# gregorgebhardt/gym-kilobots

Measured on AMD Instinct MI355X. Metric: kilobot-steps/sec, higher is better.
Workload: dtype f32

## Files before the change

gym_kilobots_amd/csrc/kb_regsolve_bins.inc:

```
{
    constexpr int KRB = KB_KREG_BINS;
    const bool solving = (int)__builtin_amdgcn_readfirstlane(wave) < nsolve;
    unsigned ra[KRB], rb[KRB], rm[KRB];
    float racc[KRB], rnx[KRB], rny[KRB];
    const unsigned WOFF = 8u * (unsigned)(NB - 5);
    char *const velB = reinterpret_cast<char *>(vel), *const posB = reinterpret_cast<char *>(pos);
#define RB_WALL(j) (ra[j] >= WOFF)
#define RB_WALLIDX(j) ((int)((ra[j] - WOFF) >> 3))
#define RB_VEL(off) (*reinterpret_cast<float2 *>(velB + (off)))
#define RB_POS(off) (*reinterpret_cast<float2 *>(posB + (off)))
#define RB_C(j) ((int)(rm[j] & 0xFFFu))
#define RB_DEPTH(j) ((int)((rm[j] >> 12) & 0x1FFu))
#define RB_FLIP(j) (((rm[j] >> 21) & 1u) != 0u)
#define RB_ISL(j) ((int)(rm[j] >> 22))
#pragma unroll
    for (int j = 0; j < KRB; ++j) { ra[j] = 0u; rb[j] = 0u; rm[j] = 0u; racc[j] = 0.0f; rnx[j] = 1.0f; rny[j] = 0.0f; }
    unsigned long long slotLevels[KRB];
    int dlo[KRB], dhi[KRB];
#pragma unroll
    for (int j = 0; j < KRB; ++j) { slotLevels[j] = 0ull; dlo[j] = 1; dhi[j] = 0; }
    int maxD = 0;
    unsigned mycnt = 0;
    const float nm_bb = p.nm_bb, nm_wb = p.nm_wb;
#ifdef KB_SOLVER_PRIO
// ... 54 lines not shown
            if (mycnt > 64u) { rlo = wave_or(rlo); rhi = wave_or(rhi); restmask = ((unsigned long long)rhi << 32) | rlo; }
        }
        wave_sync();
#ifdef KB_PROFILE
        if (tid == 0) { atomicAdd(&KB_PROF(8), (unsigned)__popcll(keymask)); atomicAdd(&KB_PROF(11), 1u); }
#endif
        KB_STAMP_PRE(19);
        unsigned *bodyDepth = islCnt;
        {
            char *const bdB = reinterpret_cast<char *>(bodyDepth);
#define RB_BD(off) (*reinterpret_cast<unsigned *>(bdB + (off)))
            unsigned rc[KRB], ia4[KRB], ib4[KRB];
#pragma unroll
            for (int j = 0; j < KRB; ++j) {
                const unsigned key = lk[j] & 63u, r = (lk[j] >> 8) & 0xFFu;
                const bool on = (lk[j] >> 31) != 0u && key != 63u;
                rc[j] = on ? ((key % RK) == RK - 1 ? (key | (r << 6)) : key) : 0xFFFFFFFFu;
                ib4[j] = 4u * (unsigned)RB_B(j);
                ia4[j] = RB_A(j) < WALL_CODE ? 4u * (unsigned)RB_A(j) : ib4[j];
            }
            const unsigned mrow = bkMaxRank[wave * NUM_CLS + min((int)lane, NUM_CLS - 1)];
            for (unsigned long long m_ = keymask; m_; m_ &= m_ - 1) {
                const unsigned key_ = (unsigned)__builtin_ctzll(m_);
                const bool rest_ = ((restmask >> key_) & 1ull) != 0ull;
                auto depth_round = [&](unsigned code_) __attribute__((always_inline)) {
#pragma unroll
                    for (int j = 0; j < KRB; ++j) {
                        if (j == 0 || rest_) {
                            if (rc[j] == code_) {
                                const unsigned d = max(RB_BD(ia4[j]), RB_BD(ib4[j])) + 1u;
                                rdepth[j] = (int)d;
                                RB_BD(ib4[j]) = d;
                                RB_BD(ia4[j]) = d;
                            }
                        }
                    }
                    wave_sync();
                };
                if ((key_ % RK) < RK - 1) depth_round(key_);
                else {
                    const unsigned maxr_ = (unsigned)__builtin_amdgcn_readlane((int)mrow, (int)(key_ / RK));
                    for (unsigned r_ = RK - 1; r_ <= maxr_; ++r_) depth_round(key_ | (r_ << 6));
                }
            }
#undef RB_BD
        }
#pragma unroll
        for (int j = 0; j < KRB; ++j) maxD = max(maxD, rdepth[j]);
        maxD = (int)wave_umax((unsigned)maxD);
        KB_STAMP_PRE(20);
        if (mycnt > 64u) {
            unsigned at[KRB];
#pragma unroll
            for (int j = 0; j < KRB; ++j) at[j] = 0u;
            unsigned base_ = 0;
            for (int d_ = SLEEP ? 0 : 1; d_ <= maxD; ++d_) {
#pragma unroll
                for (int j = 0; j < KRB; ++j) {
                    const bool is = (lk[j] >> 31) && rdepth[j] == d_;
                    const unsigned long long m_ = __ballot(is);
                    const unsigned mine = __builtin_amdgcn_mbcnt_hi((unsigned)(m_ >> 32), __builtin_amdgcn_mbcnt_lo((unsigned)m_, base_));
                    at[j] = is ? mine : at[j];
                    base_ += (unsigned)__popcll(m_);
                }
            }
#pragma unroll
            for (int j = 0; j < KRB; ++j)
                if (lk[j] >> 31) {
                    lOrder[mybase + at[j]] = (unsigned short)((lk[j] >> 16) & 0xFFFu);
                    lCbk[mybase + at[j]] = (unsigned short)rdepth[j];
                }
            wave_sync();
            unsigned short o_[KRB], l_[KRB];
#pragma unroll
            for (int j = 0; j < KRB; ++j) {
                const unsigned i_ = mybase + ((lk[j] >> 31) ? lane + 64u * j : 0u);
                o_[j] = lOrder[i_]; l_[j] = lCbk[i_];
            }
#pragma unroll
            for (int j = 0; j < KRB; ++j) {
                const bool v_ = (lk[j] >> 31) != 0u;
                lk[j] = v_ ? ((lk[j] & 0x8000FFFFu) | ((unsigned)o_[j] << 16)) : lk[j];
                rdepth[j] = v_ ? (int)l_[j] : rdepth[j];
            }
        }
        KB_STAMP_PRE(21);
#pragma unroll
        for (int j = 0; j < KRB; ++j) {
            const unsigned long long mine = (lk[j] >> 31) ? 1ull << min(rdepth[j], 63) : 0ull;
            const unsigned lo = wave_or((unsigned)mine), hi = wave_or((unsigned)(mine >> 32));
            slotLevels[j] = ((unsigned long long)hi << 32) | (unsigned long long)lo;
            const unsigned long long lv = slotLevels[j] >> 1;
            dlo[j] = lv ? (int)__builtin_ctzll(lv) + 1 : 1;
            dhi[j] = lv ? ((lv >> 62) ? maxD : 64 - (int)__builtin_clzll(lv)) : 0;
        }
        {
            unsigned c_[KRB], pr_[KRB], inf_[KRB], root_[KRB];
            float acc_[KRB];
            float2 pa_[KRB], pb_[KRB];
            bool v_[KRB];
#pragma unroll
            for (int j = 0; j < KRB; ++j) {
                v_[j] = (lk[j] >> 31) != 0u;
                c_[j] = v_[j] ? (lk[j] >> 16) & 0xFFFu : 0u;
                pr_[j] = lPair[c_[j]]; inf_[j] = lInfo[c_[j]]; acc_[j] = lAcc[c_[j]];
            }
#pragma unroll
            for (int j = 0; j < KRB; ++j) {
                pr_[j] = v_[j] ? pr_[j] : 0u;
                const int a = (int)(pr_[j] & 0xFFFFu), b = (int)(pr_[j] >> 16);
                pa_[j] = pos[a >= WALL_CODE ? b : a]; pb_[j] = pos[b]; root_[j] = parent[b];
            }
            bool pairOn[KRB];
            float dx[KRB], dy[KRB], dd[KRB], wnx[KRB], wny[KRB];
            bool ieee = false;
#pragma unroll
            for (int j = 0; j < KRB; ++j) {
                const int a = (int)(pr_[j] & 0xFFFFu), b = (int)(pr_[j] >> 16);
                const bool wallA = a >= WALL_CODE, flip = (inf_[j] & 0x80u) != 0u;
                ra[j] = wallA ? WOFF + 8u * (unsigned)(a - WALL_CODE) : 8u * (unsigned)a;
                rb[j] = 8u * (unsigned)b;
                racc[j] = v_[j] ? acc_[j] : 0.0f;
                rm[j] = v_[j] ? (c_[j] | ((unsigned)rdepth[j] << 12) | (flip ? 1u << 21 : 0u) | (root_[j] << 22)) : 0u;
                float dist;
                wall_geom(p, wallA ? a - WALL_CODE : 0, pb_[j].x, pb_[j].y, dist, wnx[j], wny[j]);
                if (flip) { wnx[j] = -wnx[j]; wny[j] = -wny[j]; }
                dx[j] = pb_[j].x - pa_[j].x; dy[j] = pb_[j].y - pa_[j].y;
                dd[j] = dx[j] * dx[j] + dy[j] * dy[j];
                pairOn[j] = v_[j] && !wallA && dd[j] > B2_EPSILON * B2_EPSILON;
                ieee = ieee || (pairOn[j] && !kb_exact_guard(dd[j]));
                if (wallA) { rnx[j] = wnx[j]; rny[j] = wny[j]; } else { rnx[j] = 1.0f; rny[j] = 0.0f; }
            }
            if (__builtin_expect(__builtin_amdgcn_ballot_w64(ieee) == 0ull, 1)) {
#pragma unroll
                for (int j = 0; j < KRB; ++j) {
                    const float len = kb_sqrt_refine(dd[j], __builtin_amdgcn_sqrtf(dd[j]), __builtin_amdgcn_rsqf(dd[j]));
                    const float inv = kb_rcp_refine(len, __builtin_amdgcn_rcpf(len));
                    if (pairOn[j]) { rnx[j] = dx[j] * inv; rny[j] = dy[j] * inv; }
                }
            } else {
#pragma unroll
                for (int j = 0; j < KRB; ++j) {
                    const float len = sqrtf(dd[j]);
                    const float inv = 1.0f / len;
                    if (pairOn[j]) { rnx[j] = dx[j] * inv; rny[j] = dy[j] * inv; }
                }
            }
        }
#undef RB_A
#undef RB_B
#ifdef KB_PROFILE
        if (lane == 0) atomicMax(&misc[M_PROF], (unsigned)maxD);
        if (tid == 0) atomicAdd(&KB_PROF(M_PROF_DEPTH), (unsigned)maxD);
        KB_STAMP(7);
#endif
    }
    KB_ABLATE_EXIT(9);
#define RB_ON(j) (RB_DEPTH(j) == d_)
    if (solving) {
#pragma unroll
        for (int j = 0; j < KRB; ++j) {
            for (int d_ = dlo[j]; d_ <= dhi[j]; ++d_) {
                if (RB_ON(j)) {
                    const float2 va = RB_VEL(ra[j]), vb = RB_VEL(rb[j]);
                    const float Px = racc[j] * rnx[j], Py = racc[j] * rny[j];
                    const float ima = RB_WALL(j) ? 0.0f : p.im_bot;
                    RB_VEL(ra[j]) = make_float2(va.x - ima * Px, va.y - ima * Py);
                    RB_VEL(rb[j]) = make_float2(vb.x + p.im_bot * Px, vb.y + p.im_bot * Py);
                }
                wave_sync();
            }
        }
        KB_STAMP_PRE(29);
    }
    KB_ABLATE_EXIT(10);
    if (solving) {
        for (int it = 0; it < p.vel_iters; ++it) {
#pragma unroll
            for (int j = 0; j < KRB; ++j) {
                for (int d_ = dlo[j]; d_ <= dhi[j]; ++d_) {
                    if (RB_ON(j)) {
                        const float2 va = RB_VEL(ra[j]), vb = RB_VEL(rb[j]);
                        const bool wallA = RB_WALL(j);
                        const float nx = rnx[j], ny = rny[j];
                        const float ima = wallA ? 0.0f : p.im_bot, imb = p.im_bot;
                        const float dvx = vb.x - va.x, dvy = vb.y - va.y;
                        const float vn = dvx * nx + dvy * ny;
                        float lambda = -((wallA ? nm_wb : nm_bb) * vn);
                        const float accOld = racc[j];
                        const float newimp = fmaxf(accOld + lambda, 0.0f);
                        lambda = newimp - accOld;
                        racc[j] = newimp;
                        const float Px = lambda * nx, Py = lambda * ny;
                        RB_VEL(ra[j]) = make_float2(va.x - ima * Px, va.y - ima * Py);
                        RB_VEL(rb[j]) = make_float2(vb.x + imb * Px, vb.y + imb * Py);
                    }
                    wave_sync();
                }
            }
        }
        KB_STAMP_PRE(30);
    }
    KB_STAMP(4);
    KB_RETID();
    KB_ABLATE_EXIT(11);
    if (solving) {
#pragma unroll
        for (int j = 0; j < KRB; ++j)
            if (lane + 64u * j < mycnt) lAcc[RB_C(j)] = racc[j];
    }
    {
        const unsigned char unsolved = (unsigned char)(p.pos_iters <= 0 ? 1 : 0);
        char *const sxB = reinterpret_cast<char *>(startX), *const syB = reinterpret_cast<char *>(startY);
        auto integrate_xy = [&](const unsigned off8, const float2 v0, const float2 p0) __attribute__((always_inline)) {
            float vxx = v0.x, vyy = v0.y;
            *reinterpret_cast<float *>(sxB + (off8 >> 1)) = p0.x; *reinterpret_cast<float *>(syB + (off8 >> 1)) = p0.y;
            const float tx = h * vxx, ty = h * vyy;
            if (tx * tx + ty * ty > B2_MAX_TRANSLATION_SQ) {
                const float ratio = B2_MAX_TRANSLATION / sqrtf(tx * tx + ty * ty);
                vxx *= ratio; vyy *= ratio;
            }
            RB_POS(off8) = make_float2(p0.x + h * vxx, p0.y + h * vyy);
            RB_VEL(off8) = make_float2(vxx, vyy);
        };
        bool intA[KRB], intB[KRB], own[BPT];
        {
            unsigned dA[KRB], dB[KRB], mk[BPT];
            const char *const bdB = reinterpret_cast<const char *>(islCnt);
#pragma unroll
            for (int j = 0; j < KRB; ++j) {
                dA[j] = *reinterpret_cast<const unsigned *>(bdB + ((RB_WALL(j) ? rb[j] : ra[j]) >> 1));
                dB[j] = *reinterpret_cast<const unsigned *>(bdB + (rb[j] >> 1));
            }
#pragma unroll
            for (int q = 0; q < BPT; ++q) mk[q] = intMark[(unsigned)ms[q] & 31u];
#pragma unroll
            for (int j = 0; j < KRB; ++j) {
                const unsigned d = (unsigned)RB_DEPTH(j);
                intA[j] = solving && d != 0u && !RB_WALL(j) && dA[j] == d;
                intB[j] = solving && d != 0u && dB[j] == d;
            }
#pragma unroll
            for (int q = 0; q < BPT; ++q) {
                own[q] = tid + q * nt < N && ((mk[q] >> ((unsigned)ms[q] >> 5)) & 1u) == 0u;
            }
        }
        wave_sync();
        static_assert(KRB == BPT, "a register slot and a kilobot of the owner thread share a trip");
#pragma unroll
        for (int j = 0; j < KRB; ++j) {
            const unsigned oo = 8u * (unsigned)ms[j];
            const float2 vO = RB_VEL(oo), pO = RB_POS(oo);
            const unsigned char aO = SLEEP ? active[ms[j]] : (unsigned char)1;
            if (j == 0 || mycnt > 64u) {
                const float2 vA = RB_VEL(ra[j]), vB = RB_VEL(rb[j]), pA = RB_POS(ra[j]), pB = RB_POS(rb[j]);
                if (intA[j]) {
                    integrate_xy(ra[j], vA, pA);
                    if (SLEEP) islWave[ra[j] >> 3] = (unsigned char)(2 | unsolved);
                }
                if (intB[j]) {
                    integrate_xy(rb[j], vB, pB);
                    if (SLEEP) islWave[rb[j] >> 3] = (unsigned char)(2 | unsolved);
                }
            }
            if (own[j]) {
                integrate_xy(oo, vO, pO);
                if (SLEEP) islWave[ms[j]] = (unsigned char)((aO ? 2 : 0) | unsolved);
            }
            float ww = bw[j];
            const float rot = h * ww;
            if (rot * rot > B2_MAX_ROTATION_SQ) {
                const float ratio = B2_MAX_ROTATION / fabsf(rot);
                ww *= ratio;
            }
            th[j] += h * ww;
            bw[j] = ww;
        }
    }
    wave_sync();
    KB_STAMP(5);
    KB_ABLATE_EXIT(12);
    if (solving) {
        for (int it = 0; it < p.pos_iters; ++it) {
            unsigned char *act = active + (it & 1) * NB, *nxt = active + ((it + 1) & 1) * NB;
            bool viol = false;
            bool ron[KRB];
#pragma unroll
            for (int j = 0; j < KRB; ++j) ron[j] = (lane + 64u * j < mycnt) && act[RB_ISL(j)] != 0;
#pragma unroll
            for (int j = 0; j < KRB; ++j) {
                for (int d_ = dlo[j]; d_ <= dhi[j]; ++d_) {
                    if (ron[j] && RB_ON(j)) {
                    const bool wallA = RB_WALL(j);
                    const int isl = RB_ISL(j);
                    float nx, ny, sep;
                    const float ima = wallA ? 0.0f : p.im_bot, imb = p.im_bot;
                    const float2 pb = RB_POS(rb[j]);
                    const float bx = pb.x, by = pb.y;
                    float axx = 0.0f, ayy = 0.0f;
                    if (wallA) {
                        float dist, wx, wy;
                        wall_geom(p, RB_WALLIDX(j), bx, by, dist, wx, wy);
                        nx = RB_FLIP(j) ? -wx : wx; ny = RB_FLIP(j) ? -wy : wy;
                        const float along = RB_FLIP(j) ? -dist : dist;
                        sep = along - B2_POLYGON_RADIUS - p.r_bot;
                    } else {
// ... 50 lines not shown
```

gym_kilobots_amd/csrc/kb_step_kernel.h:

```cpp
#pragma once
#include <utility>

#include "kb_common.h"
#include "kb_objects.h"

namespace kb {

template <int DRIVE_MODE, int LIGHT_TYPE, bool OBJ, int FN = 0, int TIER = 0, bool POLY = true, bool SENSE = true, bool SLEEP = false>
__global__ void __launch_bounds__(TIER == 1 ? 64 : 64 * KB_MAX_WAVES, (TIER == 1 || TIER == 3) ? 2 : ((TIER == 2 || (FN != 0 && !OBJ)) ? KB_COMPACT_WAVES_PER_SIMD : KB_MIN_WAVES_PER_SIMD)) kb_step_kernel(const Params p) {
    constexpr bool WIDE = TIER == 1 || TIER == 3;
    constexpr bool BINS = !OBJ;
    constexpr int KRX = BINS ? KB_KREG_BINS : KREG;
    constexpr bool PAR_DS = FN != 0 && BINS;
    static_assert(!SLEEP || FN == 0 || !OBJ, "the fixed-size instantiations with objects do not carry the sleep state");
    extern __shared__ __align__(16) unsigned char smem[];
    {
        static_assert(sizeof(Params) >= 6 * 64, "the six lines asked for are kernel arguments");
        const __attribute__((address_space(4))) unsigned *ka_ = (const __attribute__((address_space(4))) unsigned *)__builtin_amdgcn_kernarg_segment_ptr();
        const __attribute__((address_space(1))) unsigned char *m_ = (const __attribute__((address_space(1))) unsigned char *)p.env_mask;
        asm volatile("" : "+s"(m_) : "s"(ka_[0]), "s"(ka_[16]), "s"(ka_[32]), "s"(ka_[48]), "s"(ka_[64]), "s"(ka_[80]));
        if (m_ && !m_[blockIdx.x]) return;
    }
    int e = blockIdx.x;
    int tid = threadIdx.x;
// ... 934 lines not shown
                        for (int w2 = 0; w2 < 3; ++w2) {
                            float dist, nx, ny;
                            wall_geom(p, w2, ax, ay, dist, nx, ny);
                            if (w2 < wl && !(dist * dist > rw2)) r++;
                        }
                        cls = CLS_WALL | (int)(inf0 & 0x80u);
                        slot = nbots + r;
                        acc = ws_find(a, (unsigned)(WALL_CODE + wl));
                    } else {
                        const int a = pr & 0xFFFF;
                        const unsigned b = pr >> 16;
                        const int cell = cellOf[a];
                        const int cx = cell % p.gw, cy = cell / p.gw;
                        const float ax = pos[a].x, ay = pos[a].y;
                        if (k == 0) cls = CLS_SAME;
                        else if (k == 1) cls = CLS_E + (cx & 1);
                        else if (k == 2) cls = CLS_N + (cy & 1);
                        else if (k == 3) cls = CLS_NE + (cx & 1);
                        else cls = CLS_NW + (cx & 1);
                        const unsigned dc = dirCnt[a];
                        int sbase = 0;
                        for (int k2 = 0; k2 < k; ++k2) sbase += (int)((dc >> (6 * k2)) & 63u);
                        int rbase = 0;
                        for (unsigned a2 = head[hix(cell)]; a2 != (unsigned)EMPTY16; a2 = nextb[a2])
                            if ((int)a2 < a && (!hashed || (int)cellOf[a2] == cell)) rbase += (int)((dirCnt[a2] >> (6 * k)) & 63u);
                        int j = 0;
                        if (((dc >> (6 * k)) & 63u) > 1u) {
                            const int oc = (cy + dir_dy(k)) * p.gw + (cx + dir_dx(k));
                            for (unsigned b2 = head[hix(oc)]; b2 != (unsigned)EMPTY16; b2 = nextb[b2]) {
                                if (b2 >= b || (k == 0 && (int)b2 <= a) || (hashed && (int)cellOf[b2] != oc)) continue;
                                const float2 pb2 = pos[b2];
                                const float ex = pb2.x - ax, ey = pb2.y - ay;
                                if (!(ex * ex + ey * ey > rr2)) j++;
                            }
                        }
                        r = rbase + j;
                        slot = sbase + j;
                        acc = ws_find(a, b);
                        if (acc < 0.0f) acc = ws_find((int)b, (unsigned)a);
                        unsigned ra = a, rb = b;
                        for (;;) {
                            while (true) { unsigned t = lds_load_relaxed<PAR_DS>(&parent[ra]); if (t == ra) break; ra = t; }
                            while (true) { unsigned t = lds_load_relaxed<PAR_DS>(&parent[rb]); if (t == rb) break; rb = t; }
                            if (ra == rb) break;
                            if (ra < rb) { unsigned t = ra; ra = rb; rb = t; }
                            if (atomicCAS(&parent[ra], ra, rb) == ra) break;
                        }
                    }
                    if (acc < 0.0f) acc = 0.0f;
                    if (slot >= S) slot = 255;
                    if (r > 255) { r = 255; atomicOr(&misc[M_STATUS], 4u); }
                    sInfo[c] = (unsigned)cls | ((unsigned)r << 8) | ((unsigned)slot << 16) | fixbits;
                    sAcc[c] = acc;
                }
            };
            if (big) label_pass(gPair, gInfo, gAcc); else label_pass(lPair, lInfo, lAcc);
            KB_STAMP_PRE(18);
            __syncthreads();
            KB_STAMP(2);
            KB_RETID();

        }

        if (SLEEP) {
#pragma unroll
            for (int q = 0; q < BPT; ++q) {
                const int b = tid + q * nt;
                if (b >= N) continue;
                const int cnt = wsCnt[b], off = wsOff[b];
                for (int s_ = 0; s_ < cnt && off + s_ < p.cap; ++s_) {
                    const float a_ = oldInLds ? oldAcc[off + s_] : g.ws_acc[wo + off + s_];
                    if (a_ < 0.0f) continue;
                    unsigned key = oldInLds ? (unsigned)oldKey[off + s_] : g.ws_key[wo + off + s_];
                    if (!oldInLds) key = key >= KEY_OBJ ? OBJ_CODE + (key - KEY_OBJ) : (key >= KEY_WALL ? WALL_CODE + (key - KEY_WALL) : key);
                    if (key >= (unsigned)WALL_CODE) continue;
                    if (slp[q] < 0.0f) slp[q] = 0.0f;
                    if (key >= (unsigned)OBJ_CODE) {
                        if (OBJ) { const int m_ = ot_body(objTab + (key - OBJ_CODE) * OT_WORDS); if (objSlp[m_] < 0.0f) objSlp[m_] = 0.0f; }
                    } else atomicOr(&misc[M_WAKE + (key >> 5)], 1u << (key & 31u));
                }
            }
            __syncthreads();
#pragma unroll
            for (int q = 0; q < BPT; ++q) {
                const int b = tid + q * nt;
                if (b < N && slp[q] < 0.0f && ((misc[M_WAKE + (b >> 5)] >> (b & 31)) & 1u)) slp[q] = 0.0f;
            }
        }
        for (int b = tid; b < N; b += nt) {
            unsigned r = b;
            while (true) { unsigned t = lds_load_relaxed<PAR_DS>(&parent[r]); if (t == r) break; r = t; }
            parent[b] = r;
            islCnt[b] = 0;
            islWave[b] = (unsigned char)((unsigned)b % (unsigned)nsolve);
            if (!BINS) head[hix(cellOf[b])] = EMPTY16;
            if (!SLEEP) active[b] = 1;
            active[NB + b] = 0;
            if (!BINS && SENSE && p.sense_s > 0 && drive) g.nbr_count[o + b] = (unsigned)newOff[b];
        }
        if (tid < 64) bkStart[tid] = 0;
        if (tid < 32) bkFill[tid] = 0;
        if (tid < M) {
            const int b = N + tid;
            unsigned r = b;
            while (true) { unsigned t = lds_load_relaxed<PAR_DS>(&parent[r]); if (t == r) break; r = t; }
            parent[b] = r;
            islCnt[b] = 0;
            islWave[b] = (unsigned char)((unsigned)b % (unsigned)nw);
            if (!SLEEP) active[b] = 1;
            active[NB + b] = 0;
        }
        if (SLEEP && !BINS) {
#pragma unroll
            for (int q = 0; q < BPT; ++q) {
                const int b = tid + q * nt;
                if (b < N && !(slp[q] < 0.0f)) active[parent[b]] = 1;
            }
            if (tid < M && !(objSlp[tid] < 0.0f)) active[parent[N + tid]] = 1;
        }
        if (BINS) __syncthreads();
        else newTotal = block_scan_u8(wsCntNew, newOff, NP, wsum, tid);
        if (SLEEP && BINS) {
#pragma unroll
            for (int q = 0; q < BPT; ++q) {
                const int b = tid + q * nt;
                if (b < N && !(slp[q] < 0.0f)) active[parent[ms[q]]] = 1;
            }
        }
        const bool newInLds = BINS ? !big : newTotal <= (unsigned)capL_;
        if (OBJ && wave == 0) {
            unsigned root = 0;
            const bool on = lane < NMC && mcTouch;
            if (on) { root = parent[mci(ox, MC_B, lane)]; mci_set(ox, MC_ISL, lane, (int)root); }
        }
        KB_STAMP(14);
        KB_RETID();
        KB_ABLATE_EXIT(7);
        const bool wcntDead = BINS && nw > 1 && p.solver_mode == 0;
        auto census = [&](const unsigned *sPair) __attribute__((always_inline)) {
            for (int c = tid; c < ncon; c += nt) {
                const unsigned root = parent[sPair[c] >> 16];
                const unsigned n = atomicAdd(&islCnt[root], 1u) + 1u;
                if (n > (unsigned)GIANT_ISLAND) atomicMax(&misc[M_MAXISL], n);
                if (!wcntDead) atomicAdd(&misc[M_WCNT + islWave[root]], 1u);
            }
        };
        if (big) census(gPair); else census(lPair);
        __syncthreads();
        unsigned maxw = 0;
        for (int w = 0; w < nw; ++w) maxw = max(maxw, misc[M_WCNT + w]);
        bool coopForced = misc[M_MAXISL] > (unsigned)GIANT_ISLAND || p.solver_mode == 2 || p.solver_mode == 4;
        bool coop = coopForced || nw == 1;
        if (!coop && !big && p.solver_mode == 0) {
            unsigned *szSum = bkStart, *szPre = bkStart + 32, *szFill = bkFill;
            for (int b = tid; b < N + M; b += nt) {
                if (parent[b] != (unsigned)b) continue;
                const unsigned cnt_ = islCnt[b];
                if (cnt_ != 0) atomicAdd(&szSum[32u - min(cnt_, 32u)], cnt_);
            }
            __syncthreads();
            if (wave == 0) {
                const unsigned v_ = lane < 32 ? szSum[lane] : 0u;
                const unsigned incl = wave_incl_scan(v_);
                if (lane < 32) szPre[lane] = incl - v_;
                if (lane < nw) misc[M_WCNT + lane] = 0;
            }
            __syncthreads();
            unsigned chunk = 60u;
            if ((unsigned)ncon > 60u * (unsigned)(nw - 1) + 124u) chunk = ((unsigned)ncon - 124u + (unsigned)nw - 2u) / (unsigned)(nw - 1);
            if (BINS) chunk = ((unsigned)ncon + (unsigned)nsolve - 1u) / (unsigned)nsolve;
            for (int b = tid; b < N + M; b += nt) {
                if (parent[b] != (unsigned)b) continue;
                const unsigned cnt_ = islCnt[b];
                if (cnt_ == 0) continue;
                const unsigned q_ = 32u - min(cnt_, 32u);
                const unsigned at = szPre[q_] + atomicAdd(&szFill[q_], cnt_);
                const unsigned w_ = min(at / max(chunk, 1u), (unsigned)nsolve - 1u);
                islWave[b] = (unsigned char)w_;
                atomicAdd(&misc[M_WCNT + w_], cnt_);
            }
            __syncthreads();
            maxw = 0;
            for (int w = 0; w < nw; ++w) maxw = max(maxw, misc[M_WCNT + w]);
        }
        bool reg = !coopForced && !big && maxw <= 64u * KRX && p.solver_mode == 0;
        if (!coop && !big && maxw > 64u * KRX && p.solver_mode == 0) {
            unsigned short *bigList = bkList;
            __syncthreads();
            if (tid < nw) misc[M_WCNT + tid] = 0;
            if (tid == 0) misc[M_TOTAL] = 0;
            __syncthreads();
            for (int b = tid; b < N + M; b += nt) {
                if (parent[b] != (unsigned)b) continue;
                const unsigned cnt_ = islCnt[b];
                if (cnt_ == 0) continue;
                unsigned slot_ = 64u;
                if (cnt_ >= (unsigned)BIG_ISLAND) slot_ = atomicAdd(&misc[M_TOTAL], 1u);
                if (slot_ < 64u) bigList[slot_] = (unsigned short)b;
                else atomicAdd(&misc[M_WCNT + islWave[b]], cnt_);
            }
            __syncthreads();
            if (wave == 0) {
                const int nb = (int)min(misc[M_TOTAL], 64u);
                const unsigned root = lane < nb ? (unsigned)bigList[lane] : 0u;
                const unsigned size = lane < nb ? islCnt[root] : 0u;
                int rank = 0;
                for (int j = 0; j < nb; ++j) {
                    const unsigned sj = __shfl(size, j), rj = __shfl(root, j);
                    if (sj > size || (sj == size && rj < root)) rank++;
                }
                unsigned load = lane < nsolve ? misc[M_WCNT + lane] : 0u;
                int myWave = 0;
                for (int r = 0; r < nb; ++r) {
                    const int src = __builtin_ctzll(__ballot(lane < nb && rank == r));
                    const unsigned sz = __shfl(size, src);
                    unsigned key = lane < nsolve ? ((load << 4) | (unsigned)lane) : 0xFFFFFFFFu;
                    for (int d = 8; d >= 1; d >>= 1) key = min(key, __shfl_xor(key, d));
                    const int wmin = (int)(__shfl(key, 0) & 15u);
                    if (lane == wmin) load += sz;
                    if (lane == src) myWave = wmin;
                }
                if (lane < nb) islWave[root] = (unsigned char)myWave;
                if (lane < nsolve) misc[M_WCNT + lane] = load;
            }
            __syncthreads();
            maxw = 0;
            for (int w = 0; w < nw; ++w) maxw = max(maxw, misc[M_WCNT + w]);
            reg = maxw <= 64u * KRX;
        }
        if (BINS && nw > 1 && !reg && p.solver_mode == 0) { coopForced = true; coop = true; }
        if (OBJ && wave == 0) {
            const bool on = lane < NMC && mcTouch && (!SLEEP || active[mci(ox, MC_ISL, lane)] != 0);
            const unsigned w_ = on ? (unsigned)islWave[mci(ox, MC_ISL, lane)] : 0u;
            for (int w = 0; w < nw; ++w) {
                const unsigned long long mk = __ballot(on && (int)w_ == w);
                if (lane == 0) mcMask[w] = mk;
            }
            const unsigned long long all = __ballot(on);
            if (lane == 0) mcMask[nw] = all;
        }
        auto mc_warm_pass = [&](unsigned long long mask, bool leader) __attribute__((always_inline)) {
            if (leader) for (unsigned long long m_ = mask; m_; m_ &= m_ - 1) mc_warm_start(ox, __builtin_ctzll(m_));
        };
        auto mc_velocity_pass = [&](unsigned long long mask, bool leader) __attribute__((always_inline)) {
            if (leader) for (unsigned long long m_ = mask; m_; m_ &= m_ - 1) mc_solve_velocity(ox, __builtin_ctzll(m_));
        };
        auto mc_position_pass = [&](unsigned long long mask, bool leader, const unsigned char *act, unsigned char *nxt, bool lastIt) __attribute__((always_inline)) -> bool {
            bool viol = false;
            if (leader)
                for (unsigned long long m_ = mask; m_; m_ &= m_ - 1) {
                    const int t = __builtin_ctzll(m_);
                    const int isl = mci(ox, MC_ISL, t);
                    if (!act[isl]) continue;
                    const float minSep = mc_solve_position(ox, t, B2_BAUMGARTE);
                    if (minSep < -3.0f * B2_LINEAR_SLOP) { nxt[isl] = 1; viol = true; if (SLEEP && lastIt) islWave[isl] = 3; }
                }
            return viol;
        };
        auto mc_clear_flags = [&](unsigned long long mask, bool leader, unsigned char *act) __attribute__((always_inline)) {
            if (leader) for (unsigned long long m_ = mask; m_; m_ &= m_ - 1) act[mci(ox, MC_ISL, __builtin_ctzll(m_))] = 0;
        };
        auto mc_store = [&]() __attribute__((always_inline)) {
            if (OBJ && wave == 0 && lane < NMC) {
                int owner, col;
                mc_candidate(F, lane, owner, col);
                float *dst = owsMine + (owner * KB_OWS_COLS + col) * KB_OWS_WORDS;
                float o[KB_OWS_WORDS] = {-1.0f, -1.0f, -1.0f, -1.0f, -1.0f, -1.0f};
                if (mcTouch) {
                    const int cnt = (mci(ox, MC_TYPE, lane) >> 2) & 3, ids = mci(ox, MC_ID, lane);
                    o[0] = (float)(ids & 255); o[1] = mcf(ox, MC_NI0, lane); o[2] = mcf(ox, MC_TI0, lane);
                    if (cnt == 2) { o[3] = (float)((ids >> 8) & 255); o[4] = mcf(ox, MC_NI1, lane); o[5] = mcf(ox, MC_TI1, lane); }
                }
#pragma unroll
                for (int k = 0; k < KB_OWS_WORDS; ++k) dst[k] = o[k];
            }
        };
        auto bucket_sort = [&](const unsigned *sPair, const unsigned *sInfo, unsigned short *cbk,
                               unsigned short *order) __attribute__((always_inline)) {
            const int W = coop ? 1 : nw;
            for (int b = tid; b < N + M; b += nt) islCnt[b] = 0;
            for (int k = tid; k < W * BK_PER_WAVE; k += nt) { bkStart[k] = 0; bkFill[k] = 0; }
            for (int k = tid; k < W * NUM_CLS; k += nt) bkMaxRank[k] = 0;
            if (tid == 0) bkStart[W * BK_PER_WAVE] = 0;
            __syncthreads();
            for (int c = tid; c < ncon; c += nt) {
                const unsigned root = parent[sPair[c] >> 16];
                if (SLEEP && !active[root]) { cbk[c] = EMPTY16; continue; }
                const int w = coop ? 0 : (int)islWave[root];
                const unsigned inf = sInfo[c];
                const int cls = inf & 0x7F, r = (inf >> 8) & 0xFF;
                const int bk = (w * NUM_CLS + cls) * RK + (r < RK - 1 ? r : RK - 1);
                cbk[c] = (unsigned short)bk;
                atomicAdd(&bkStart[bk], 1u);
                if (r >= RK - 1) atomicMax(&bkMaxRank[w * NUM_CLS + cls], (unsigned)r);
            }
            __syncthreads();
            if (wave == 0) {
                const int nb = W * BK_PER_WAVE;
                const int chunk = (nb + 63) / 64;
                const int s0 = lane * chunk, e0 = min(nb, s0 + chunk);
                unsigned sum = 0;
                for (int i = s0; i < e0; ++i) sum += bkStart[i];
                const unsigned incl = wave_incl_scan(sum);
                unsigned run = incl - sum;
                for (int i = s0; i < e0; ++i) { unsigned v = bkStart[i]; bkStart[i] = run; run += v; }
                if (lane == 63) bkStart[nb] = incl;
            }
            __syncthreads();
            for (int c = tid; c < ncon; c += nt) {
                const int bk = cbk[c];
                if (SLEEP && bk == (int)EMPTY16) continue;
                order[bkStart[bk] + atomicAdd(&bkFill[bk], 1u)] = (unsigned short)c;
            }
            if (wave < W) {
                const int base = wave * BK_PER_WAVE;
                const bool ne = lane < BK_PER_WAVE && bkStart[base + lane + 1] > bkStart[base + lane];
                const unsigned long long m = __ballot(ne);
                if (ne) bkList[base + __popcll(m & ((1ull << lane) - 1ull))] = (unsigned short)(base + lane);
                if (lane == 0) nList[wave] = (unsigned char)__popcll(m);
            }
            __syncthreads();
        };
        if (reg) {
            for (int b = tid; b < N + M; b += nt) islCnt[b] = 0;
            if (tid < nw * NUM_CLS) bkMaxRank[tid] = 0;
            if constexpr (BINS) {
                if (tid < 32) intMark[tid] = 0;
                if (wave_s == 0) {
                    const unsigned v_ = lane < nw ? misc[M_WCNT + lane] : 0u;
                    const unsigned incl = wave_incl_scan(v_);
                    if (lane < nw) misc[M_WFILL + lane] = incl - v_;
                }
// ... 680 lines not shown
                mc_store();
                const bool last = sub == p.n_substeps - 1;
                for (int c = tid; c < (BINS ? 0 : ncon); c += nt) {
                    const unsigned inf = sInfo[c];
                    const int sl = (inf >> 16) & 0xFF;
                    if (sl == 255) continue;
                    const unsigned pr = sPair[c];
                    const int a = pr & 0xFFFF, b = pr >> 16;
                    const int owner = a < WALL_CODE ? a : b;
                    const float acc = sAcc[c];
                    const unsigned key16 = a >= WALL_CODE ? (unsigned)a : (b >= N ? (unsigned)OBJ_CODE + ((inf >> 24) & 15u) : (unsigned)b);
                    const unsigned pos = (unsigned)newOff[owner] + (unsigned)sl;
                    if (pos >= (unsigned)p.cap) continue;
                    if (newInLds) { oldKey[pos] = (unsigned short)key16; oldAcc[pos] = acc; }
                    if (last || !newInLds) {
                        g.ws_key[wo + pos] = key16 >= (unsigned)WALL_CODE ? KEY_WALL + (key16 - WALL_CODE)
                                           : (key16 >= (unsigned)OBJ_CODE ? KEY_OBJ + (key16 - OBJ_CODE) : key16);
                        g.ws_acc[wo + pos] = acc;
                    }
                }
#pragma unroll
                for (int q = 0; q < BPT; ++q) {
                    const int b_ = tid + q * nt;
                    if (b_ >= N) continue;
                    const int b = KB_SLOT(q, b_);
                    float vxx = vel[b].x, vyy = vel[b].y, ww = bw[q];
                    if (BINS) { startX[b] = pos[b].x; startY[b] = pos[b].y; }
                    const float tx = h * vxx, ty = h * vyy;
                    if (tx * tx + ty * ty > B2_MAX_TRANSLATION_SQ) {
                        const float ratio = B2_MAX_TRANSLATION / sqrtf(tx * tx + ty * ty);
                        vxx *= ratio; vyy *= ratio;
                    }
                    const float rot = h * ww;
                    if (rot * rot > B2_MAX_ROTATION_SQ) {
                        const float ratio = B2_MAX_ROTATION / fabsf(rot);
                        ww *= ratio;
                    }
                    pos[b].x += h * vxx; pos[b].y += h * vyy;
                    th[q] += h * ww;
                    vel[b].x = vxx; vel[b].y = vyy; bw[q] = ww;
                    if (SLEEP) islWave[b] = (unsigned char)((active[b] ? 2 : 0) | (p.pos_iters <= 0 ? 1 : 0));
                }
                if (tid < M) {
                    const int b = N + tid;
                    float vxx = vel[b].x, vyy = vel[b].y, ww = objW[tid];
                    const float tx = h * vxx, ty = h * vyy;
                    if (tx * tx + ty * ty > B2_MAX_TRANSLATION_SQ) {
                        const float ratio = B2_MAX_TRANSLATION / sqrtf(tx * tx + ty * ty);
                        vxx *= ratio; vyy *= ratio;
                    }
                    const float rot = h * ww;
                    if (rot * rot > B2_MAX_ROTATION_SQ) ww *= B2_MAX_ROTATION / fabsf(rot);
                    vel[b].x = vxx; vel[b].y = vyy; objW[tid] = ww;
                    pos[b].x += h * vxx; pos[b].y += h * vyy;
                    objA[tid] += h * ww;
                    if (SLEEP) islWave[b] = (unsigned char)((active[b] ? 2 : 0) | (p.pos_iters <= 0 ? 1 : 0));
                }
                __syncthreads();
                KB_STAMP(5);
                KB_RETID();
                for (int it = 0; it < p.pos_iters; ++it) {
                    unsigned char *act = active + (it & 1) * NB, *nxt = active + ((it + 1) & 1) * NB;
                    bool viol = false;
                    KB_FOR_ROUNDS(false, false, {
                        const unsigned pr = KB_PR;
                        const int a = pr & 0xFFFF, b = pr >> 16;
                        const int isl = (int)parent[b];
                        if (act[isl] && bpoly(b)) {
                            const int m = b - N;
                            const float *T = objTab + ((KB_INF >> 24) & 15u) * OT_WORDS;
                            V2 ln, lp;
                            collide_poly_circle(T, xf_of_body(objBody + m * BT_WORDS, start[b].x, start[b].y, objA0[m]), mk2(start[a].x, start[a].y), p.r_bot, ln, lp);
                            const XF xo = body_xf(ox, b);
                            const V2 normal = rot_mul(xo, ln);
                            const V2 planePoint = xf_mul(xo, lp);
                            const V2 clipPoint = mk2(pos[a].x, pos[a].y);
                            const float sep = v_dot(v_sub(clipPoint, planePoint), normal) - T[OT_RADIUS] - p.r_bot;
                            const V2 rA = v_sub(clipPoint, mk2(pos[b].x, pos[b].y));
                            if (sep < -3.0f * B2_LINEAR_SLOP) { nxt[isl] = 1; viol = true; if (SLEEP && it == p.pos_iters - 1) islWave[isl] = 3; }
                            const float C = kb_clampf(B2_BAUMGARTE * (sep + B2_LINEAR_SLOP), -B2_MAX_LINEAR_CORRECTION, 0.0f);
                            const float rnA = v_cross(rA, normal);
                            const float K = T[OT_IM] + KB_IM_BOT(a) + T[OT_II] * rnA * rnA;
                            const float imp = K > 0.0f ? -C / K : 0.0f;
                            const V2 P = v_scale(imp, normal);
                            pos[b].x -= T[OT_IM] * P.x; pos[b].y -= T[OT_IM] * P.y;
                            objA[m] -= T[OT_II] * v_cross(rA, P);
                            pos[a].x += KB_IM_BOT(a) * P.x; pos[a].y += KB_IM_BOT(a) * P.y;
                        } else if (act[isl]) {
                            float nx, ny, sep;
                            const float ima = bim(a), imb = bim(b), rda = brad(a), rdb = brad(b);
                            const float bx = pos[b].x, by = pos[b].y;
                            float axx = 0.0f, ayy = 0.0f;
                            if (a >= WALL_CODE) {
                                float dist, wx, wy;
                                wall_geom(p, a - WALL_CODE, bx, by, dist, wx, wy);
                                const bool flipped = (KB_INF & 0x80) != 0;
                                nx = flipped ? -wx : wx; ny = flipped ? -wy : wy;
                                const float along = flipped ? -dist : dist;
                                sep = along - rda - rdb;
                            } else {
                                axx = pos[a].x; ayy = pos[a].y;
                                const float dx = bx - axx, dy = by - ayy;
                                const float len = sqrtf(dx * dx + dy * dy);
                                nx = dx; ny = dy;
                                if (!(len < B2_EPSILON)) { const float inv = 1.0f / len; nx = dx * inv; ny = dy * inv; }
                                sep = (dx * nx + dy * ny) - rda - rdb;
                            }
                            if (sep < -3.0f * B2_LINEAR_SLOP) { nxt[isl] = 1; viol = true; if (SLEEP && it == p.pos_iters - 1) islWave[isl] = 3; }
                            const float C = kb_clampf(B2_BAUMGARTE * (sep + B2_LINEAR_SLOP), -B2_MAX_LINEAR_CORRECTION, 0.0f);
                            const float K = ima + imb;
                            const float imp = K > 0.0f ? -C / K : 0.0f;
                            const float Px = imp * nx, Py = imp * ny;
                            if (a < WALL_CODE) { pos[a].x = axx - ima * Px; pos[a].y = ayy - ima * Py; }
                            pos[b].x = bx + imb * Px; pos[b].y = by + imb * Py;
                        }
                    })
                    if (OBJ && myMc) { viol |= mc_position_pass(myMc, leader, act, nxt, it == p.pos_iters - 1); KB_ROUND_SYNC(); }
#ifdef KB_PROFILE
                    if (tid == 0) atomicAdd(&KB_PROF(10), 1u);
#endif
                    bool any;
                    if (coop) {
                        if (viol) misc[M_ANY] = 1u;
                        __syncthreads();
                        any = misc[M_ANY] != 0u;
                        __syncthreads();
                        if (tid == 0) misc[M_ANY] = 0u;
                    } else {
                        any = __any(viol);
                    }
                    if (!any) break;
                    {
                        const int s_ = (int)bkStart[myw * BK_PER_WAVE], e_ = (int)bkStart[(myw + 1) * BK_PER_WAVE];
                        for (int i_ = s_ + lid; i_ < e_; i_ += stride) act[parent[sPair[order[i_]] >> 16]] = 0;
                        if (OBJ && myMc) mc_clear_flags(myMc, leader, act);
                    }
                    KB_ROUND_SYNC();
                }
#undef KB_FOR_ROUNDS
#undef KB_FOR_ROUNDS_PF
#undef KB_FOR_ROUNDS_PLAIN
#undef KB_VEL_NORMAL
#undef KB_ROUND_SYNC
            };
            if (big) {
                float *gN = reinterpret_cast<float *>(g.scratch) + (size_t)p.E * p.cap * 4 + wo * 3;
                solve_list(gPair, gInfo, gAcc, gCbk, gOrder, gN, true);
            } else solve_list(lPair, lInfo, lAcc, lCbk, lOrder, nullptr, false);
        }
        __syncthreads();
        KB_STAMP_PRE(25);
#ifdef KB_PROFILE
        if (BINS && reg && tid == 0) atomicAdd(&KB_PROF(9), misc[M_PROF]);
#endif
        KB_RETID();
        KB_ABLATE_EXIT(13);
        if (SLEEP) {
            unsigned *islMin = BINS ? reinterpret_cast<unsigned *>(smem + (FN ? ldsb::binE(NB, NP, false, capL_) : p.islmin_off)) : lPair;
            const float linTolSqr = B2_LINEAR_SLEEP_TOL * B2_LINEAR_SLEEP_TOL, angTolSqr = B2_ANGULAR_SLEEP_TOL * B2_ANGULAR_SLEEP_TOL;
            for (int b = tid; b < N + M; b += nt) islMin[b] = 0x7F7FFFFFu;
            __syncthreads();
#pragma unroll
            for (int q = 0; q < BPT; ++q) {
                const int b_ = tid + q * nt;
                if (b_ >= N) continue;
                const int b = KB_SLOT(q, b_);
                const unsigned r = parent[b];
                if (!(islWave[r] & 2)) continue;
                if (slp[q] < 0.0f) slp[q] = 0.0f;
                const float2 v_ = vel[b];
                if (bw[q] * bw[q] > angTolSqr || v_.x * v_.x + v_.y * v_.y > linTolSqr) { slp[q] = 0.0f; atomicMin(&islMin[r], 0u); }
                else { slp[q] += h; atomicMin(&islMin[r], __float_as_uint(slp[q])); }
            }
            if (tid < M) {
                const int b = N + tid;
                const unsigned r = parent[b];
                if (islWave[r] & 2) {
                    float sl = objSlp[tid];
                    if (sl < 0.0f) sl = 0.0f;
                    const float2 v_ = vel[b];
                    const float w_ = objW[tid];
                    if (w_ * w_ > angTolSqr || v_.x * v_.x + v_.y * v_.y > linTolSqr) { sl = 0.0f; atomicMin(&islMin[r], 0u); }
                    else { sl += h; atomicMin(&islMin[r], __float_as_uint(sl)); }
                    objSlp[tid] = sl;
                }
            }
            __syncthreads();
#pragma unroll
            for (int q = 0; q < BPT; ++q) {
                const int b_ = tid + q * nt;
                if (b_ >= N) continue;
                const int b = KB_SLOT(q, b_);
                const unsigned r = parent[b];
                const unsigned st_ = islWave[r];
                if ((st_ & 2) && !(st_ & 1) && __uint_as_float(islMin[r]) >= B2_TIME_TO_SLEEP) {
                    slp[q] = -1.0f; vel[b].x = 0.0f; vel[b].y = 0.0f; bw[q] = 0.0f;
                }
            }
            if (tid < M) {
                const int b = N + tid;
                const unsigned r = parent[b];
                const unsigned st_ = islWave[r];
                if ((st_ & 2) && !(st_ & 1) && __uint_as_float(islMin[r]) >= B2_TIME_TO_SLEEP) {
                    objSlp[tid] = -1.0f; vel[b].x = 0.0f; vel[b].y = 0.0f; objW[tid] = 0.0f;
                }
            }
            __syncthreads();
        }
        bool toiRecords = false;
        if (p.toi_walls) {
            float *cTh0 = reinterpret_cast<float *>(BINS ? parent : lInfo), *cTh = BINS ? reinterpret_cast<float *>(lPair) : lAcc;
            float *cW = reinterpret_cast<float *>(BINS ? lOrder : lCbk);
            unsigned short *cSlot = reinterpret_cast<unsigned short *>(active);
            const int candMax = BINS ? min(capL_, N) : capL_ / 2;
            int cand[BPT];
            if (!BINS) {
                if (tid == 0) misc[M_NCON] = 0;
                __syncthreads();
            }
#pragma unroll
            for (int q = 0; q < BPT; ++q) {
                const int b_ = tid + q * nt;
                cand[q] = -1;
                if (b_ >= N) continue;
                const int b = KB_SLOT(q, b_);
                if (SLEEP && slp[q] < 0.0f) continue;
                const float xa = BINS ? startX[b] : start[b].x, ya = BINS ? startY[b] : start[b].y, xb = pos[b].x, yb = pos[b].y;
                bool none = true;
#pragma unroll
                for (int wl = 0; wl < 4; ++wl) none &= kb_toi_no_event(p, wl, p.toi_tt, xa, ya, xb, yb);
                if (none) continue;
                const int i = (int)atomicAdd(&misc[M_NCON], 1u);
                if (i >= candMax) { atomicOr(&misc[M_STATUS], 8u); continue; }
                cand[q] = i;
                if (BINS) cSlot[i] = (unsigned short)b; else lPair[i] = (unsigned)b;
                cTh0[i] = sth0[q]; cTh[i] = th[q]; cW[i] = bw[q];
            }
            __syncthreads();
            KB_STAMP_PRE(26);
            const int ncand = min((int)misc[M_NCON], candMax);
            toiRecords = OBJ || ncand > 0;
            if (toiRecords) {
                for (int i = tid; i < ncand; i += nt) {
                    const int b = BINS ? (int)cSlot[i] : (int)lPair[i];
                    float R = p.r_bot, im = KB_IM_BOT(b);
                    asm volatile("" : "+v"(R), "+v"(im));
                    float x_ = pos[b].x, y_ = pos[b].y, a_ = cTh[i], vx_ = vel[b].x, vy_ = vel[b].y, w_ = cW[i];
                    kb_toi_walls_body(p, R, im, BINS ? startX[b] : start[b].x, BINS ? startY[b] : start[b].y, cTh0[i], x_, y_, a_, vx_, vy_, w_);
                    pos[b].x = x_; pos[b].y = y_; vel[b].x = vx_; vel[b].y = vy_; cTh[i] = a_; cW[i] = w_;
                }
                if (OBJ && tid < M && !(SLEEP && objSlp[tid] < 0.0f)) {
                    Arena ar;
                    ar.xmin = p.xmin; ar.ymin = p.ymin; ar.xmax = p.xmax; ar.ymax = p.ymax;
                    toi_walls_object(ox, ar, F, tid, start[N + tid].x, start[N + tid].y, objA0[tid], p.h, p.vel_iters,
                                     g.ows_acc + (size_t)e * (MAXOBJ * KB_OWS_COLS * KB_OWS_WORDS));
                }
                KB_STAMP_PRE(27);
                __syncthreads();
                KB_STAMP_PRE(28);
#pragma unroll
                for (int q = 0; q < BPT; ++q)
                    if (cand[q] >= 0) { th[q] = cTh[cand[q]]; bw[q] = cW[cand[q]]; }
            } else { KB_STAMP_PRE(27); KB_STAMP_PRE(28); }
        }
        KB_ABLATE_EXIT(14);
        if (OBJ && tid < M && sub + 1 < p.n_substeps &&
            (objBody[tid * BT_WORDS + BT_LCX] != 0.0f || objBody[tid * BT_WORDS + BT_LCY] != 0.0f)) {
            const XF t0 = body_xf(ox, N + tid);
            const XF t1 = xf_make(t0.p.x, t0.p.y, objA[tid]);
            const V2 cm = xf_mul(t1, mk2(objBody[tid * BT_WORDS + BT_LCX], objBody[tid * BT_WORDS + BT_LCY]));
            pos[N + tid].x = cm.x; pos[N + tid].y = cm.y;
        }
        const bool lastSub = sub == p.n_substeps - 1;
        if (PARK && !lastSub) {
#pragma unroll
            for (int q = 0; q < BPT; ++q) {
                const int b = tid + q * nt;
                if (b < N) vel[b] = make_float2(g.v[o + b], g.w[o + b]);
            }
        }
        if (!lastSub) for (int b = tid; b < NP; b += nt) { wsCnt[b] = wsCntNew[b]; wsOff[b] = newOff[b]; }
        if (BINS) {
            if (toiRecords && !lastSub) __syncthreads();
            const int nlist = (int)min(newTotal, (unsigned)stageCap);
            auto list_out = [&](const unsigned *sInfo, const float *sAcc) __attribute__((always_inline)) {
                for (int i = tid; i < nlist; i += nt) {
                    const unsigned key16 = sInfo[i] >> 16;
                    const float acc = sAcc[i];
                    if (newInLds && !lastSub) { oldKey[i] = (unsigned short)key16; oldAcc[i] = acc; }
                    if (lastSub || !newInLds) {
                        g.ws_key[wo + i] = key16 >= (unsigned)WALL_CODE ? KEY_WALL + (key16 - WALL_CODE) : key16;
                        g.ws_acc[wo + i] = acc;
                    }
                }
            };
            if (big) list_out(gInfo, gAcc); else list_out(lInfo, lAcc);
            if (!lastSub) for (int c = tid; c < ldsb::bin_entries(p.nhead) / 2; c += nt) reinterpret_cast<unsigned *>(E1)[c] = 0u;
        }
        oldInLds = newInLds;
        oldTotal = newTotal;
        if (!lastSub) __syncthreads();
        KB_STAMP(6);
    }

    KB_ENV_ADDRESSES();
#pragma unroll
// ... 65 lines not shown
```

Before: 16.94 billion.

## Pack islands into solver waves by register capacity instead of even contact chunks

For the bins path, the island-to-wave assignment now computes per-wave start boundaries in a single wave-level scan over size classes. Each wave is filled up to 64 or 128 contacts (one or two register slots) without splitting islands, falling back to the even split only when capacity runs out. The aim is to keep more waves on the register solver path and cut the number of depth rounds per wave. The cost is extra serial scan work in wave 0 before the assignment loop. Profiling counters for rounds and overflow are also added under KB_PROFILE.

```diff
diff --git a/gym_kilobots_amd/csrc/kb_regsolve_bins.inc b/gym_kilobots_amd/csrc/kb_regsolve_bins.inc
--- a/gym_kilobots_amd/csrc/kb_regsolve_bins.inc
+++ b/gym_kilobots_amd/csrc/kb_regsolve_bins.inc
@@ -230,6 +230,13 @@
 #ifdef KB_PROFILE
         if (lane == 0) atomicMax(&misc[M_PROF], (unsigned)maxD);
         if (tid == 0) atomicAdd(&KB_PROF(M_PROF_DEPTH), (unsigned)maxD);
+        {
+            unsigned rounds_ = 0;
+#pragma unroll
+            for (int j = 0; j < KRB; ++j) rounds_ += dhi[j] >= dlo[j] ? (unsigned)(dhi[j] - dlo[j] + 1) : 0u;
+            if (lane == 0) { if (mycnt > 64u) atomicAdd(&KB_PROF(36), 16u); atomicMax(&KB_PROF(38), rounds_); }
+            if (tid == 0) atomicAdd(&KB_PROF(39), 16u * rounds_);
+        }
         KB_STAMP(7);
 #endif
     }
diff --git a/gym_kilobots_amd/csrc/kb_step_kernel.h b/gym_kilobots_amd/csrc/kb_step_kernel.h
--- a/gym_kilobots_amd/csrc/kb_step_kernel.h
+++ b/gym_kilobots_amd/csrc/kb_step_kernel.h
@@ -1110,7 +1110,8 @@
         bool coopForced = misc[M_MAXISL] > (unsigned)GIANT_ISLAND || p.solver_mode == 2 || p.solver_mode == 4;
         bool coop = coopForced || nw == 1;
         if (!coop && !big && p.solver_mode == 0) {
-            unsigned *szSum = bkStart, *szPre = bkStart + 32, *szFill = bkFill;
+            unsigned *szSum = bkStart, *szPre = bkStart + 32, *szFill = bkFill, *szTab = bkFill + 32;
+            static_assert(MAX_WAVES <= 32 && lds::nbk(2) >= 32 + MAX_WAVES, "szTab: a word per wave behind the 32 class counters");
             for (int b = tid; b < N + M; b += nt) {
                 if (parent[b] != (unsigned)b) continue;
                 const unsigned cnt_ = islCnt[b];
@@ -1121,21 +1122,71 @@
                 const unsigned v_ = lane < 32 ? szSum[lane] : 0u;
                 const unsigned incl = wave_incl_scan(v_);
                 if (lane < 32) szPre[lane] = incl - v_;
-                if (lane < nw) misc[M_WCNT + lane] = 0;
+                if constexpr (BINS) {
+                    const unsigned excl = incl - v_;
+                    const unsigned s_ = 32u - min(lane, 31u);
+                    const unsigned mg_ = (unsigned)(65536.5f * __builtin_amdgcn_rcpf((float)s_)) + 1u;
+                    const unsigned total = (unsigned)__builtin_amdgcn_readlane((int)incl, 31);
+                    bool even = __builtin_amdgcn_readfirstlane((int)v_) != 0;
+                    bool two = false;
+                    unsigned pos = 0, first = lane == 0u ? 0u : total;
+                    if (!even) {
+#pragma unroll
+                        for (unsigned w = 0; w < (unsigned)nsolve; ++w) {
+                            if (pos >= total) break;
+                            const unsigned s = 32u - (unsigned)__builtin_ctzll(__ballot(incl > pos));
+                            two = two || total - pos + s > ((unsigned)nsolve - 1u - w) * (129u - s) + 65u;
+                            const unsigned end = pos + (two ? 128u : 64u);
+                            const unsigned long long m_ = __ballot(incl > end);
+                            unsigned nxt = total;
+                            if (m_ != 0ull) {
+                                const int q = __builtin_ctzll(m_);
+                                const unsigned start = max(pos, (unsigned)__builtin_amdgcn_readlane((int)excl, q));
+                                nxt = start + (((end - start) * (unsigned)__builtin_amdgcn_readlane((int)mg_, q)) >> 16) * (32u - (unsigned)q);
+                            }
+                            first = lane == w + 1u ? nxt : first;
+                            pos = nxt;
+                        }
+                        even = pos < total;
+                    }
+                    const unsigned mine = even ? 0u : (unsigned)__shfl_down((int)first, 1) - first;
+                    if (even) first = lane * max(((unsigned)ncon + (unsigned)nsolve - 1u) / (unsigned)nsolve, 1u);
+                    if (lane >= (unsigned)nsolve) first = 0xFFFFFFFFu;
+                    if (lane < MAX_WAVES) szTab[lane] = lane == 0u ? (even ? 1u : 0u) : first;
+                    if (lane < nw) misc[M_WCNT + lane] = mine;
+                } else if (lane < nw) misc[M_WCNT + lane] = 0;
             }
             __syncthreads();
-            unsigned chunk = 60u;
-            if ((unsigned)ncon > 60u * (unsigned)(nw - 1) + 124u) chunk = ((unsigned)ncon - 124u + (unsigned)nw - 2u) / (unsigned)(nw - 1);
-            if (BINS) chunk = ((unsigned)ncon + (unsigned)nsolve - 1u) / (unsigned)nsolve;
-            for (int b = tid; b < N + M; b += nt) {
-                if (parent[b] != (unsigned)b) continue;
-                const unsigned cnt_ = islCnt[b];
-                if (cnt_ == 0) continue;
-                const unsigned q_ = 32u - min(cnt_, 32u);
-                const unsigned at = szPre[q_] + atomicAdd(&szFill[q_], cnt_);
-                const unsigned w_ = min(at / max(chunk, 1u), (unsigned)nsolve - 1u);
-                islWave[b] = (unsigned char)w_;
-                atomicAdd(&misc[M_WCNT + w_], cnt_);
+            if constexpr (BINS) {
+                unsigned st_[MAX_WAVES];
+#pragma unroll
+                for (int k = 0; k < MAX_WAVES; ++k) st_[k] = szTab[k];
+                const bool even = st_[0] != 0u;
+                for (int b = tid; b < N + M; b += nt) {
+                    if (parent[b] != (unsigned)b) continue;
+                    const unsigned cnt_ = islCnt[b];
+                    if (cnt_ == 0) continue;
+                    const unsigned q_ = 32u - min(cnt_, 32u);
+                    const unsigned at = szPre[q_] + atomicAdd(&szFill[q_], cnt_);
+                    unsigned w_ = 0;
+#pragma unroll
+                    for (int k = 1; k < MAX_WAVES; ++k) w_ += at >= st_[k] ? 1u : 0u;
+                    islWave[b] = (unsigned char)w_;
+                    if (even) atomicAdd(&misc[M_WCNT + w_], cnt_);
+                }
+            } else {
+                unsigned chunk = 60u;
+                if ((unsigned)ncon > 60u * (unsigned)(nw - 1) + 124u) chunk = ((unsigned)ncon - 124u + (unsigned)nw - 2u) / (unsigned)(nw - 1);
+                for (int b = tid; b < N + M; b += nt) {
+                    if (parent[b] != (unsigned)b) continue;
+                    const unsigned cnt_ = islCnt[b];
+                    if (cnt_ == 0) continue;
+                    const unsigned q_ = 32u - min(cnt_, 32u);
+                    const unsigned at = szPre[q_] + atomicAdd(&szFill[q_], cnt_);
+                    const unsigned w_ = min(at / max(chunk, 1u), (unsigned)nsolve - 1u);
+                    islWave[b] = (unsigned char)w_;
+                    atomicAdd(&misc[M_WCNT + w_], cnt_);
+                }
             }
             __syncthreads();
             maxw = 0;
@@ -2122,6 +2173,7 @@
         KB_STAMP_PRE(25);
 #ifdef KB_PROFILE
         if (BINS && reg && tid == 0) atomicAdd(&KB_PROF(9), misc[M_PROF]);
+        if (BINS && reg && tid == 0) { atomicAdd(&KB_PROF(37), 16u * KB_PROF(38)); KB_PROF(38) = 0u; }
 #endif
         KB_RETID();
         KB_ABLATE_EXIT(13);
```

After: 17.33 billion (median of 6 runs). 2.3% higher.
